# krullgit/3D-Object-Detection-for-autonomous-navigation

Measured on AMD Instinct MI355X. Metric: frames/sec (whole node) + p50 per-frame ms, 16k-pt pillars, higher is better.
Workload: dtype f32 (GEMMs on the 16-bit matrix pipe as split operands -- two float16 pieces per value, 3 products, fp32 accumulate: fp32-equivalent results, measured 1.5e-6 max from the fp32 oracle at this shape)

## Files before the change

### 3d-object-detection-for-autonomous-navigation_amd/csrc/backbone.hip

```cpp
#include <stdio.h>
#include <stdlib.h>
#include <string.h>

#include "pp_common.h"
#include "pp_plan.h"

typedef float f32x16 __attribute__((ext_vector_type(16)));
typedef _Float16 f16x8 __attribute__((ext_vector_type(8)));
#define PC_MFMA(A, B, C) __builtin_amdgcn_mfma_f32_32x32x16_f16(A, B, C, 0, 0, 0)
#define PC_PRODUCTS(ACC, XH, XM, YH, YM) \
    ACC = PC_MFMA(XM, YH, ACC); ACC = PC_MFMA(XH, YM, ACC); ACC = PC_MFMA(XH, YH, ACC);
typedef unsigned u32x4 __attribute__((ext_vector_type(4)));

__device__ __forceinline__ float4 buf_load16(__amdgpu_buffer_rsrc_t r, unsigned voff, unsigned soff) {
    const u32x4 v = __builtin_amdgcn_raw_buffer_load_b128(r, voff, soff, 0);
    return make_float4(__uint_as_float(v.x), __uint_as_float(v.y), __uint_as_float(v.z), __uint_as_float(v.w));
}
__device__ __forceinline__ void buf_store16(float4 v, __amdgpu_buffer_rsrc_t r, unsigned voff, unsigned soff) {
    const u32x4 u = {__float_as_uint(v.x), __float_as_uint(v.y), __float_as_uint(v.z), __float_as_uint(v.w)};
    __builtin_amdgcn_raw_buffer_store_b128(u, r, voff, soff, 0);
}
__device__ __forceinline__ __amdgpu_buffer_rsrc_t make_rsrc(const void* base) {
    return __builtin_amdgcn_make_buffer_rsrc(const_cast<void*>(base), 0, 0x7ffffffe, 0x00020000);
}

#define PX_TILE 128

#define KC 32
#define LDS_STRIDE 36

struct GemmArgs {
    const float* in;
    const float* dw;
    const float* wt;
    const unsigned short* wt16;
    int n_total;
    const float* bias;
    float* out;
    float* head;
    const float* head_wt;
    const float* head_wt16;
    const float* head_bias;
    int head_mode;
    int M;
    int tile_lo;
    int in_h, in_w, cin;
    int px_h, px_w;
    int stride;
    int ld_out, co_off;
    int epi;
    int k, cout;
    const int* occ;
    int occ_nz;
    const unsigned long long* occbits;
    int occ_w64;
    float* cls_plane;
    int cls_col0, cls_ncol;
    const float4* tr_coef;
    float* tr_D;
    float* tr_stat;
};

template <int NTILES>
__device__ __forceinline__ void gemm_epilogue(const GemmArgs& a, f32x16 (&acc)[NTILES], int p0, int n0, int wave,
                                              int lane, const int* s_opix) {
    const int h = lane >> 5, col_l = lane & 31;
    if (a.epi == 0) {
#pragma unroll
        for (int n = 0; n < NTILES; ++n) {
            const int col = n0 + n * 32 + col_l;
            const float bv = a.bias[col];
            float* dst = a.out + a.co_off + col;
#pragma unroll
            for (int r = 0; r < 16; ++r) {
                const int pix = p0 + wave * 32 + (r & 3) + 8 * (r >> 2) + 4 * h;
                if (pix < a.M) dst[(size_t)pix * a.ld_out] = relu_keep_nan(acc[n][r] + bv);
            }
        }
    } else if (a.epi == 1) {
        const int k = a.k, OW = a.px_w * k;
#pragma unroll
        for (int n = 0; n < NTILES; ++n) {
            const int col0 = __builtin_amdgcn_readfirstlane(n0 + n * 32);
            const int tap = col0 / a.cout, co = col0 - tap * a.cout + col_l;
            const int i = tap / k, j = tap - i * k;
            const int delta = i * OW + j;
            const float bv = a.bias[co];
            float* dst = a.out + a.co_off + co;
#pragma unroll
            for (int r = 0; r < 16; ++r) {
                const int row = wave * 32 + (r & 3) + 8 * (r >> 2) + 4 * h;
                if (p0 + row < a.M) dst[(size_t)(s_opix[row] + delta) * a.ld_out] = relu_keep_nan(acc[n][r] + bv);
            }
        }
    } else {
        const int col = n0 + col_l;
        const float bv = a.bias[col];
#pragma unroll
        for (int r = 0; r < 16; ++r) {
            const int pix = p0 + wave * 32 + (r & 3) + 8 * (r >> 2) + 4 * h;
            if (pix < a.M) a.head[(size_t)pix * PP_HEAD_COLS + col] = acc[0][r] + bv;
        }
    }
}

template <int NT, int MODE>
__global__ __launch_bounds__(256) void k_gemm_layer(GemmArgs a) {
    __shared__ __attribute__((aligned(16))) float sA[PX_TILE * LDS_STRIDE];
    __shared__ __attribute__((aligned(16))) float sB[NT * LDS_STRIDE];
    __shared__ int s_opix[PX_TILE];
    constexpr int NTILES = NT / 32;

    const int tid = threadIdx.x, lane = tid & 63, wave = tid >> 6;
    int mt;
    {
        const int nwg = gridDim.x, orig = blockIdx.x;
        const int q = nwg >> 3, r = nwg & 7, xcd = orig & 7;
        mt = ((xcd < r) ? xcd * (q + 1) : r * (q + 1) + (xcd - r) * q) + (orig >> 3);
    }
    const int p0 = mt * PX_TILE;
    const int n0 = blockIdx.y * NT;
    const int cin = a.cin;
    if (a.epi == 1 && tid < PX_TILE) {
        const int pix = min(p0 + tid, a.M - 1);
        const int hw = a.px_h * a.px_w;
        const int b = pix / hw, rem = pix - b * hw;
        const int y = rem / a.px_w, x = rem - y * a.px_w;
        s_opix[tid] = (b * a.px_h * a.k + y * a.k) * (a.px_w * a.k) + x * a.k;
    }

    const int c4 = tid & 7;
    const float* ibase[4];
    int yi0[4], xi0[4];
    bool pvalid[4];
    {
        const int hw = a.px_h * a.px_w;
#pragma unroll
        for (int it = 0; it < 4; ++it) {
            const int pix = p0 + (tid >> 3) + 32 * it;
            pvalid[it] = pix < a.M;
            const int pc = pvalid[it] ? pix : 0;
            const int b = pc / hw;
            const int rem = pc - b * hw;
            const int yo = rem / a.px_w, xo = rem - yo * a.px_w;
            if (MODE == 0) {
                yi0[it] = yo * a.stride - 1;
                xi0[it] = xo * a.stride - 1;
                ibase[it] = a.in + (size_t)b * a.in_h * a.in_w * cin;
            } else {
                yi0[it] = 0; xi0[it] = 0;
                ibase[it] = a.in + (size_t)pc * cin;
            }
        }
    }

    f32x16 acc[NTILES];
#pragma unroll
    for (int n = 0; n < NTILES; ++n)
#pragma unroll
        for (int r = 0; r < 16; ++r) acc[n][r] = 0.f;
// ... 1315 lines not shown
}

template <int NT, int WPS>
__global__ __launch_bounds__(256, WPS) void k_deconv_u(GemmArgs a, int ntiles) {
    constexpr int KCH = 16;
    constexpr int NTILES = NT / 32;
    constexpr int SB = PP_NPIECE * NT * 8;
    constexpr int NBI = NT * 2 * PP_NPIECE;
    constexpr int NB4 = (NBI + 255) / 256;
    constexpr int SHW = (NT / 16) * PP_NPIECE * 32 * 8;
    __shared__ __attribute__((aligned(16))) float sB[2 * SB];
    __shared__ __attribute__((aligned(16))) float sHW[SHW];
    __shared__ float s_bias[NT];
    __shared__ float s_hbias[PP_HEAD_COLS];
    __shared__ int s_opix[2][128];
    const int tid = threadIdx.x, lane = tid & 63, wave = tid >> 6;
    const int h = lane >> 5, r32 = lane & 31;

    const int xcd = blockIdx.x & 7, gl = blockIdx.x >> 3, GL = gridDim.x >> 3;
    const int tbase = (int)(((long long)xcd * ntiles) >> 3), tend = (int)(((long long)(xcd + 1) * ntiles) >> 3);
    const int first = tbase + gl;
    if (first >= tend) return;
    const int ntl = (tend - first + GL - 1) / GL;
    const int n0 = blockIdx.y * NT;
    const int cin = a.cin;
    const int nchunks = cin / KCH;
    const int total = ntl * nchunks;
    const int tap = n0 / a.cout, cbase = n0 - tap * a.cout;
    const int ti = tap / a.k;
    const int delta = ti * (a.px_w * a.k) + (tap - ti * a.k);
    const bool heads = a.head_mode != 0;

    const int hwpx = a.px_h * a.px_w;
#define D_FILL_OPIX(TILE, SLOT)                                                         \
    if (tid < 128) {                                                                    \
        const int pix_ = min((TILE) * 128 + tid, a.M - 1);                              \
        const int b_ = pix_ / hwpx, rem_ = pix_ - b_ * hwpx;                            \
        const int y_ = rem_ / a.px_w, x_ = rem_ - y_ * a.px_w;                          \
        s_opix[SLOT][tid] = (b_ * a.px_h * a.k + y_ * a.k) * (a.px_w * a.k) + x_ * a.k; \
    }
    D_FILL_OPIX(first, 0)

    const __amdgpu_buffer_rsrc_t rs_in = make_rsrc(reinterpret_cast<const char*>(a.in) - PP_ZPAD_FLOATS * 4);
    const __amdgpu_buffer_rsrc_t rs_wt = make_rsrc(a.wt16);
    unsigned boff[NB4];
    int bdst[NB4];
#pragma unroll
    for (int r = 0; r < NB4; ++r) {
        const int e_ = (tid + 256 * r) % NBI;
        const int piece = e_ / (NT * 2), rem = e_ % (NT * 2), row = rem >> 1, half = rem & 1;
        boff[r] = (unsigned)(((piece * a.n_total + n0 + row) * 16 + half * 8) * 2);
        bdst[r] = piece * (NT * 8) + row * 8 + ((half ^ ((row >> 3) & 1)) * 4);
    }
    const unsigned bstep = (unsigned)(PP_NPIECE * a.n_total * 32);
    float4 rb0, rb1, rb2;
    rb0 = rb1 = rb2 = make_float4(0.f, 0.f, 0.f, 0.f);
    static_assert(NB4 <= 3, "weight prefetch registers");
#define D_LOAD_B(KCIDX)                                                                                  \
    {                                                                                                    \
        const unsigned sb_ = (unsigned)(KCIDX) * bstep;                                                  \
        if (NBI % 256 == 0 || NB4 > 1 || tid < NBI) rb0 = buf_load16(rs_wt, boff[0], sb_);               \
        if (NB4 > 1 && (NBI >= 512 || tid + 256 < NBI)) rb1 = buf_load16(rs_wt, boff[NB4 > 1 ? 1 : 0], sb_);  \
        if (NB4 > 2 && (NBI >= 768 || tid + 512 < NBI)) rb2 = buf_load16(rs_wt, boff[NB4 > 2 ? 2 : 0], sb_);  \
    }
#define D_STORE_B(BUF)                                                                                   \
    {                                                                                                    \
        if (NBI % 256 == 0 || NB4 > 1 || tid < NBI) *reinterpret_cast<float4*>(sB + (BUF) * SB + bdst[0]) = rb0;  \
        if (NB4 > 1 && (NBI >= 512 || tid + 256 < NBI)) *reinterpret_cast<float4*>(sB + (BUF) * SB + bdst[NB4 > 1 ? 1 : 0]) = rb1;  \
        if (NB4 > 2 && (NBI >= 768 || tid + 512 < NBI)) *reinterpret_cast<float4*>(sB + (BUF) * SB + bdst[NB4 > 2 ? 2 : 0]) = rb2;  \
    }
    int ld_tile = first, ld_kc = 0;
    unsigned avo = 0;
#define D_TILE_AOFF(TILE)                                                                                \
    {                                                                                                    \
        const int pix_ = (TILE) * 128 + wave * 32 + r32;                                                 \
        avo = (pix_ < a.M) ? (unsigned)(pix_ * cin + h * 8) * 4u + PP_ZPAD_FLOATS * 4u : (unsigned)(h * 32);  \
    }
#define D_LOAD_A(R0, R1)                                                                                 \
    {                                                                                                    \
        if (ld_kc == 0) D_TILE_AOFF(ld_tile)                                                             \
        const unsigned so_ = (unsigned)ld_kc * (KCH * 4);                                                \
        R0 = buf_load16(rs_in, avo, so_);                                                                \
        R1 = buf_load16(rs_in, avo + 16u, so_);                                                          \
        if (++ld_kc == nchunks) { ld_kc = 0; ld_tile += GL; }                                            \
    }
    float4 ra0, ra1, rc0, rc1;
    D_LOAD_A(ra0, ra1)
    D_LOAD_A(rc0, rc1)
    D_LOAD_B(0)
    int lb_kc = 1;
    if (tid < NT) s_bias[tid] = a.bias[cbase + tid];
    if (heads) {
        for (int e = tid; e < SHW / 4; e += 256)
            reinterpret_cast<float4*>(sHW)[e ^ ((e >> 4) & 1)] = reinterpret_cast<const float4*>(a.head_wt16)[e];
        if (tid < PP_HEAD_COLS) s_hbias[tid] = a.head_bias[tid];
    }

    int mm_tile = first, mm_kc = 0, mm_slot = 0;
    __syncthreads();
    f32x16 acc[NTILES];
#define D_INIT_ACC()                                                                                     \
    _Pragma("unroll") for (int n = 0; n < NTILES; ++n)                                                   \
        _Pragma("unroll") for (int r = 0; r < 16; ++r) acc[n][r] = s_bias[n * 32 + DCH(r, h)];
    D_INIT_ACC()
    D_STORE_B(0)
    D_LOAD_B(lb_kc)
    if (++lb_kc == nchunks) lb_kc = 0;
    __syncthreads();

#define D_STEP(I, RA0, RA1)                                                                              \
    {                                                                                                    \
        const int i_ = (I);                                                                              \
        const float av_[8] = {RA0.x, RA0.y, RA0.z, RA0.w, RA1.x, RA1.y, RA1.z, RA1.w};                   \
        f16x8 ah_, am_;                                                                                  \
        split_f16x2(av_, ah_, am_);                                                                      \
        if (i_ + 2 < total) D_LOAD_A(RA0, RA1)                                                           \
        {                                                                                                \
            const float* cB_ = sB + (i_ & 1) * SB + r32 * 8 + ((h ^ ((r32 >> 3) & 1)) * 4);              \
            _Pragma("unroll") for (int n = 0; n < NTILES; ++n) {                                         \
                const f16x8 bh_ = *reinterpret_cast<const f16x8*>(cB_ + n * 32 * 8);                     \
                const f16x8 bm_ = *reinterpret_cast<const f16x8*>(cB_ + NT * 8 + n * 32 * 8);            \
                PC_PRODUCTS(acc[n], bh_, bm_, ah_, am_)                                                  \
            }                                                                                            \
        }                                                                                                \
        if (i_ + 1 < total) D_STORE_B((i_ + 1) & 1)              \
        if (++mm_kc == nchunks) {                                                                        \
            deconv_tile_epilogue<NT>(a, acc, mm_tile, wave, lane, cbase, delta, s_opix[mm_slot], sHW, s_hbias);  \
            D_INIT_ACC()                                                                                 \
            mm_kc = 0;                                                                                   \
            mm_tile += GL;                                                                               \
            mm_slot ^= 1;                                                                                \
        } else if (mm_kc == 1 && mm_tile + GL < tend) {                                                  \
            D_FILL_OPIX(mm_tile + GL, mm_slot ^ 1)           \
        }                                                                                                \
        if (i_ + 1 < total) {    \
            if (i_ + 2 < total) D_LOAD_B(lb_kc)                                                          \
            if (++lb_kc == nchunks) lb_kc = 0;                                                           \
        }                                                                                                \
        __syncthreads();                                                                                 \
    }
    for (int i = 0; i < total; i += 2) {
        D_STEP(i, ra0, ra1)
        D_STEP(i + 1, rc0, rc1)
    }
#undef D_STEP
#undef D_INIT_ACC
#undef D_LOAD_A
#undef D_TILE_AOFF
#undef D_STORE_B
#undef D_LOAD_B
#undef D_FILL_OPIX
}

template <int CIN>
__global__ __launch_bounds__(256, 2) void k_deconv_r(GemmArgs a, int nunits, int upw) {
    constexpr int NCH = CIN / 16;
    constexpr int STEPS = 4 * NCH;
    constexpr int NPU = STEPS / 8;
    constexpr int PANEL = 8 * 2 * 256;
    constexpr int NB = 3;
    constexpr int PD = 2;
    constexpr int SHW = (128 / 16) * 2 * 32 * 8;
    static_assert(STEPS % 4 == 0 && PD < 4, "fragment ring of four");
    __shared__ __attribute__((aligned(16))) float sW[NB * PANEL];
    __shared__ __attribute__((aligned(16))) float sHW[SHW];
    __shared__ __attribute__((aligned(16))) float s_bias[128];
    __shared__ float s_hbias[PP_HEAD_COLS];
    const int tid = threadIdx.x, lane = tid & 63, wave = __builtin_amdgcn_readfirstlane(tid >> 6);
    const int h = lane >> 5, r32 = lane & 31;

    int wg;
    {
        const int G = gridDim.x, q = G >> 3, r = G & 7, xcd = blockIdx.x & 7;
        wg = (xcd < r ? xcd * (q + 1) : r * (q + 1) + (xcd - r) * q) + (blockIdx.x >> 3);
    }
    const int u0 = wg * upw, u1 = min(u0 + upw, nunits);
    if (u0 >= u1) return;
    const int ntaps = a.k * a.k;
    const bool heads = a.head_mode != 0;
    const int hwpx = a.px_h * a.px_w, OW = a.px_w * a.k;

    const __amdgpu_buffer_rsrc_t rs_in = make_rsrc(reinterpret_cast<const char*>(a.in) - PP_ZPAD_FLOATS * 4);
    const __amdgpu_buffer_rsrc_t rs_wt = make_rsrc(a.wt16);
    const int srow = lane >> 1, shalf = lane & 1;
    const unsigned wvoff = (unsigned)((((wave & 1) * a.n_total + srow) * 16 + shalf * 8) * 2);
    const int wdst = wave * 256 + srow * 8 + ((shalf ^ ((srow >> 3) & 1)) * 4);
    const unsigned cstep = (unsigned)(2 * a.n_total * 32);
    float4 rw[4];
    rw[0] = rw[1] = rw[2] = rw[3] = make_float4(0.f, 0.f, 0.f, 0.f);
    int tile = u0 / ntaps, tap = u0 - tile * ntaps;
    int ld_left = (u1 - u0) * NPU, ld_tap = tap, ld_p = 0;
#define R_LOAD_NEXT()                                                                                    \
    {                                                                                                    \
        if (ld_left > 0) {                                                                               \
            _Pragma("unroll") for (int j_ = 0; j_ < 4; ++j_) {                                           \
                const int fs_ = ld_p * 8 + (wave >> 1) + 2 * j_;                                         \
                const int nt_ = fs_ / NCH, c_ = fs_ % NCH;                                               \
                rw[j_] = buf_load16(rs_wt, wvoff, (unsigned)c_ * cstep + (unsigned)((ld_tap * 128 + nt_ * 32) * 32)); \
            }                                                                                            \
        }                                                                                                \
        --ld_left;                                                                                       \
        if (++ld_p == NPU) { ld_p = 0; if (++ld_tap == ntaps) ld_tap = 0; }                              \
    }
#define R_STORE_W(SLOT)                                                                                  \
    _Pragma("unroll") for (int j_ = 0; j_ < 4; ++j_)                                                     \
        *reinterpret_cast<float4*>(sW + (SLOT) * PANEL + wdst + j_ * 1024) = rw[j_];

    float4 ra0[NCH][2];
    const int pix0_ = tile * 128 + wave * 32 + r32;
    const bool ok0_ = pix0_ < a.M;
    {
        const unsigned avo = ok0_ ? (unsigned)(pix0_ * CIN + h * 8) * 4u + PP_ZPAD_FLOATS * 4u : (unsigned)(h * 32);
#pragma unroll
        for (int c = 0; c < NCH; ++c) {
            ra0[c][0] = buf_load16(rs_in, avo, (unsigned)c * 64u);
            ra0[c][1] = buf_load16(rs_in, avo + 16u, (unsigned)c * 64u);
        }
    }
    R_LOAD_NEXT()
    for (int e = tid; e < 128; e += 256) s_bias[e] = a.bias[e];
    if (heads) {
        for (int e = tid; e < SHW / 4; e += 256)
            reinterpret_cast<float4*>(sHW)[e ^ ((e >> 4) & 1)] = reinterpret_cast<const float4*>(a.head_wt16)[e];
        if (tid < PP_HEAD_COLS) s_hbias[tid] = a.head_bias[tid];
    }
    R_STORE_W(0)
    R_LOAD_NEXT()
    __syncthreads();

    f16x8 xh[NCH], xm[NCH];
    int tile_cur = tile, opix0;
    bool ok = ok0_;
    {
        const int pc = ok ? pix0_ : 0;
        const int pb = pc / hwpx, prem = pc - pb * hwpx;
        const int py = prem / a.px_w, pxx = prem - py * a.px_w;
        opix0 = (pb * a.px_h * a.k + py * a.k) * OW + pxx * a.k;
#pragma unroll
        for (int c = 0; c < NCH; ++c) {
            const float av[8] = {ra0[c][0].x, ra0[c][0].y, ra0[c][0].z, ra0[c][0].w, ra0[c][1].x, ra0[c][1].y, ra0[c][1].z, ra0[c][1].w};
            split_f16x2(av, xh[c], xm[c]);
        }
    }
    const float* const cW = sW + r32 * 8 + ((h ^ ((r32 >> 3) & 1)) * 4);
    const float* const cHW = sHW + r32 * 8 + ((h ^ ((r32 >> 3) & 1)) * 4);
    int slot = 0;
    const float* pcur = cW;
    const float* pnxt = cW + PANEL;
    f16x8 fh[4], fm[4];
#pragma unroll
    for (int i = 0; i < PD; ++i) {
        fh[i] = *reinterpret_cast<const f16x8*>(pcur + i * 512);
        fm[i] = *reinterpret_cast<const f16x8*>(pcur + i * 512 + 256);
    }

    constexpr bool PREF = CIN <= 128;
    float4 rn[PREF ? NCH : 1][2];
    int pre_tile = -1;
    for (int u = u0; u < u1; ++u) {
        if (tile != tile_cur) {
            tile_cur = tile;
            const int pix = tile * 128 + wave * 32 + r32;
            ok = pix < a.M;
            const unsigned avo = ok ? (unsigned)(pix * CIN + h * 8) * 4u + PP_ZPAD_FLOATS * 4u : (unsigned)(h * 32);
            float4 ra[NCH][2];
            if (PREF && pre_tile == tile) {
#pragma unroll
                for (int c = 0; c < NCH; ++c) { ra[c][0] = rn[PREF ? c : 0][0]; ra[c][1] = rn[PREF ? c : 0][1]; }
            } else {
#pragma unroll
                for (int c = 0; c < NCH; ++c) {
                    ra[c][0] = buf_load16(rs_in, avo, (unsigned)c * 64u);
                    ra[c][1] = buf_load16(rs_in, avo + 16u, (unsigned)c * 64u);
                }
            }
            const int pc = ok ? pix : 0;
            const int pb = pc / hwpx, prem = pc - pb * hwpx;
            const int py = prem / a.px_w, pxx = prem - py * a.px_w;
            opix0 = (pb * a.px_h * a.k + py * a.k) * OW + pxx * a.k;
#pragma unroll
            for (int c = 0; c < NCH; ++c) {
                const float av[8] = {ra[c][0].x, ra[c][0].y, ra[c][0].z, ra[c][0].w, ra[c][1].x, ra[c][1].y, ra[c][1].z, ra[c][1].w};
                split_f16x2(av, xh[c], xm[c]);
            }
        }
        const int ti = tap / a.k;
        const size_t orow = (size_t)(opix0 + ti * OW + (tap - ti * a.k));
        float* const hrow = a.head + orow * PP_HEAD_COLS + 4 * h;
        f32x16 hacc;
        if (a.head_mode == 2 && ok) {
#pragma unroll
            for (int g = 0; g < 4; ++g) {
                const float4 t = *reinterpret_cast<const float4*>(hrow + 8 * g);
                hacc[4 * g] = t.x; hacc[4 * g + 1] = t.y; hacc[4 * g + 2] = t.z; hacc[4 * g + 3] = t.w;
            }
        } else {
#pragma unroll
            for (int r = 0; r < 16; ++r) hacc[r] = (a.head_mode == 1) ? s_hbias[DCH(r, h)] : 0.f;
        }
        float* const dst = (a.out != nullptr) ? a.out + orow * a.ld_out + a.co_off + 4 * h : nullptr;
        f32x16 acc;
        __builtin_amdgcn_sched_barrier(0);
#pragma unroll
        for (int fs = 0; fs < STEPS; ++fs) {
            const int s = fs & 7, nt = fs / NCH, c = fs % NCH;
            if (c == 0) {
#pragma unroll
                for (int g = 0; g < 4; ++g) {
                    const float4 t = *reinterpret_cast<const float4*>(s_bias + nt * 32 + 8 * g + 4 * h);
                    acc[4 * g] = t.x; acc[4 * g + 1] = t.y; acc[4 * g + 2] = t.z; acc[4 * g + 3] = t.w;
                }
            }
            if (s == 4) __syncthreads();
            {
                const float* w_ = (s + PD < 8) ? pcur + (s + PD) * 512 : pnxt + (s + PD - 8) * 512;
                fh[(fs + PD) & 3] = *reinterpret_cast<const f16x8*>(w_);
                fm[(fs + PD) & 3] = *reinterpret_cast<const f16x8*>(w_ + 256);
            }
            PC_PRODUCTS(acc, fh[fs & 3], fm[fs & 3], xh[c], xm[c])
            if (s == 0) {
                const int ws = (slot + 1 == NB) ? 0 : slot + 1;
                R_STORE_W(ws)
            }
            if (s == 1) { R_LOAD_NEXT() }
            if (PREF && fs == 1 && tap + 1 == ntaps && u + 1 < u1) {
                pre_tile = tile + 1;
                const int pixn = pre_tile * 128 + wave * 32 + r32;
                const unsigned avn = (pixn < a.M) ? (unsigned)(pixn * CIN + h * 8) * 4u + PP_ZPAD_FLOATS * 4u : (unsigned)(h * 32);
#pragma unroll
                for (int c = 0; c < (PREF ? NCH : 0); ++c) {
                    rn[c][0] = buf_load16(rs_in, avn, (unsigned)c * 64u);
                    rn[c][1] = buf_load16(rs_in, avn + 16u, (unsigned)c * 64u);
                }
            }
            if (s == 7) {
                slot = (slot + 1 == NB) ? 0 : slot + 1;
                pcur = pnxt;
                pnxt = cW + ((slot + 1 == NB) ? 0 : slot + 1) * PANEL;
            }
            __builtin_amdgcn_sched_barrier(0);
            if (c == NCH - 1) {
                float v[16];
#pragma unroll
                for (int r = 0; r < 16; ++r) v[r] = relu_keep_nan(acc[r]);
                if (heads) {
#pragma unroll
                    for (int g = 0; g < 2; ++g) {
                        const float av[8] = {v[8 * g], v[8 * g + 1], v[8 * g + 2], v[8 * g + 3],
                                             v[8 * g + 4], v[8 * g + 5], v[8 * g + 6], v[8 * g + 7]};
                        f16x8 yh, ym;
                        split_f16x2(av, yh, ym);
                        const float* hW = cHW + (nt * 2 + g) * 2 * 32 * 8;
                        const f16x8 gh = *reinterpret_cast<const f16x8*>(hW);
                        const f16x8 gm = *reinterpret_cast<const f16x8*>(hW + 32 * 8);
                        PC_PRODUCTS(hacc, gh, gm, yh, ym)
                    }
                }
                if (dst != nullptr && ok) {
#pragma unroll
                    for (int g = 0; g < 4; ++g)
                        *reinterpret_cast<float4*>(dst + nt * 32 + 8 * g) = make_float4(v[4 * g], v[4 * g + 1], v[4 * g + 2], v[4 * g + 3]);
                }
                __builtin_amdgcn_sched_barrier(0);
            }
        }
        if (heads && ok) {
#pragma unroll
            for (int g = 0; g < 4; ++g)
                *reinterpret_cast<float4*>(hrow + 8 * g) = make_float4(hacc[4 * g], hacc[4 * g + 1], hacc[4 * g + 2], hacc[4 * g + 3]);
            if (a.cls_plane != nullptr) {
                float* cp = a.cls_plane + orow * a.cls_ncol;
#pragma unroll
                for (int r = 0; r < 16; ++r) {
                    const int col = 8 * (r >> 2) + 4 * h + (r & 3) - a.cls_col0;
                    if ((unsigned)col < (unsigned)a.cls_ncol) cp[col] = hacc[r];
                }
            }
        }
        if (++tap == ntaps) { tap = 0; ++tile; }
    }
#undef R_STORE_W
#undef R_LOAD_NEXT
}

template <int CIN>
static void launch_deconv_r(const GemmArgs& a, int cus, hipStream_t s) {
    const int ntiles = (a.M + 127) / 128;
    const long long U = (long long)ntiles * a.k * a.k;
    const int slots = 2 * cus;
    const int upw = (int)((U + slots - 1) / slots);
    const int G = (int)((U + upw - 1) / upw);
    PP_LAUNCH("k_deconv_r", (k_deconv_r<CIN>), dim3((unsigned)G), dim3(256), 0, s, a, (int)U, upw);
}

template <int NT>
__global__ __launch_bounds__(256, 2) void k_deconv_k4(GemmArgs a) {
    constexpr int KCH = 16;
    constexpr int NTILES = NT / 32;
    constexpr int SB = PP_NPIECE * NT * 8;
    constexpr int NBL = NT * 2 * PP_NPIECE / 64;
    constexpr int SHW = (NT / 16) * PP_NPIECE * 32 * 8;
    constexpr int SLOT = 16 * 64;
    constexpr int OWNERS = NTILES < 4 ? NTILES : 4;
    constexpr int SR = (4 * SB > (4 * NTILES - OWNERS) * SLOT) ? 4 * SB : (4 * NTILES - OWNERS) * SLOT;
    __shared__ __attribute__((aligned(16))) float sR[SR];
    __shared__ __attribute__((aligned(16))) float sHW[SHW];
    __shared__ float s_bias[NT];
    __shared__ float s_hbias[PP_HEAD_COLS];
    const int tid = threadIdx.x, lane = tid & 63, wave = tid >> 6;
    const int h = lane >> 5, r32 = lane & 31;
    const int n0 = blockIdx.y * NT;
    const int cin = a.cin;
    const int niter = cin / (KCH * 4);
    const int tap = n0 / a.cout, cbase = n0 - tap * a.cout;
    const int ti = tap / a.k;
    const int delta = ti * (a.px_w * a.k) + (tap - ti * a.k);
    const bool heads = a.head_mode != 0;
    float* const sBw = sR + wave * SB;

    const __amdgpu_buffer_rsrc_t rs_in = make_rsrc(reinterpret_cast<const char*>(a.in) - PP_ZPAD_FLOATS * 4);
    const __amdgpu_buffer_rsrc_t rs_wt = make_rsrc(a.wt16);
    const int pix = blockIdx.x * 32 + r32;
    const bool ok = pix < a.M;
    const unsigned avo = ok ? (unsigned)(pix * cin + h * 8) * 4u + PP_ZPAD_FLOATS * 4u : (unsigned)(h * 32);
    float4 ra[4][2];
#pragma unroll
    for (int j = 0; j < 4; ++j) {
        ra[j][0] = ra[j][1] = make_float4(0.f, 0.f, 0.f, 0.f);
        if (j < niter) {
            const unsigned so = (unsigned)(wave + 4 * j) * (KCH * 4);
            ra[j][0] = buf_load16(rs_in, avo, so);
            ra[j][1] = buf_load16(rs_in, avo + 16u, so);
        }
    }
    unsigned boff[NBL];
    int bdst[NBL];
#pragma unroll
    for (int r = 0; r < NBL; ++r) {
        const int e = lane + 64 * r;
        const int piece = e / (NT * 2), rem = e % (NT * 2), row = rem >> 1, half = rem & 1;
        boff[r] = (unsigned)(((piece * a.n_total + n0 + row) * 16 + half * 8) * 2);
        bdst[r] = piece * (NT * 8) + row * 8 + ((half ^ ((row >> 3) & 1)) * 4);
    }
    const unsigned bstep = (unsigned)(PP_NPIECE * a.n_total * 32);
    float4 rb[NBL];
#pragma unroll
    for (int r = 0; r < NBL; ++r) rb[r] = buf_load16(rs_wt, boff[r], (unsigned)wave * bstep);
    if (tid < NT) s_bias[tid] = a.bias[cbase + tid];
    if (heads) {
        for (int e = tid; e < SHW / 4; e += 256)
            reinterpret_cast<float4*>(sHW)[e ^ ((e >> 4) & 1)] = reinterpret_cast<const float4*>(a.head_wt16)[e];
        if (tid < PP_HEAD_COLS) s_hbias[tid] = a.head_bias[tid];
    }
    f32x16 acc[NTILES];
#pragma unroll
    for (int n = 0; n < NTILES; ++n)
#pragma unroll
        for (int r = 0; r < 16; ++r) acc[n][r] = 0.f;
    const float* const cB = sBw + r32 * 8 + ((h ^ ((r32 >> 3) & 1)) * 4);
#pragma unroll
    for (int j = 0; j < 4; ++j) {
        if (j < niter) {
#pragma unroll
            for (int r = 0; r < NBL; ++r) *reinterpret_cast<float4*>(sBw + bdst[r]) = rb[r];
            if (j + 1 < niter) {
#pragma unroll
                for (int r = 0; r < NBL; ++r) rb[r] = buf_load16(rs_wt, boff[r], (unsigned)(wave + 4 * (j + 1)) * bstep);
            }
            const float av[8] = {ra[j][0].x, ra[j][0].y, ra[j][0].z, ra[j][0].w, ra[j][1].x, ra[j][1].y, ra[j][1].z, ra[j][1].w};
            f16x8 ah, am;
            split_f16x2(av, ah, am);
#pragma unroll
            for (int n = 0; n < NTILES; ++n) {
                const f16x8 bh = *reinterpret_cast<const f16x8*>(cB + n * 32 * 8);
                const f16x8 bm = *reinterpret_cast<const f16x8*>(cB + NT * 8 + n * 32 * 8);
                PC_PRODUCTS(acc[n], bh, bm, ah, am)
            }
        }
    }
    auto slot = [](int w, int n) -> int {
        return w * NTILES + n - (w < OWNERS ? w : OWNERS) - ((w < OWNERS && n > w) ? 1 : 0);
    };
    __syncthreads();
#pragma unroll
    for (int n = 0; n < NTILES; ++n)
        if (n != wave) {
            float* d = sR + slot(wave, n) * SLOT + lane * 4;
#pragma unroll
            for (int g = 0; g < 4; ++g)
                *reinterpret_cast<float4*>(d + g * 256) = make_float4(acc[n][4 * g], acc[n][4 * g + 1], acc[n][4 * g + 2], acc[n][4 * g + 3]);
        }
    __syncthreads();
    const int pc = ok ? pix : 0;
    const int hwpx = a.px_h * a.px_w;
    const int pb = pc / hwpx, prem = pc - pb * hwpx;
    const int py = prem / a.px_w, pxx = prem - py * a.px_w;
    const size_t orow = (size_t)((pb * a.px_h * a.k + py * a.k) * (a.px_w * a.k) + pxx * a.k + delta);
    f32x16 hpart;
#pragma unroll
    for (int r = 0; r < 16; ++r) hpart[r] = 0.f;
    if (wave < NTILES) {
        float v[16];
#pragma unroll
        for (int n = 0; n < NTILES; ++n)
            if (n == wave) {
#pragma unroll
                for (int r = 0; r < 16; ++r) v[r] = acc[n][r];
            }
#pragma unroll
        for (int w = 0; w < 4; ++w)
            if (w != wave) {
                const float* sp = sR + slot(w, wave) * SLOT + lane * 4;
#pragma unroll
                for (int g = 0; g < 4; ++g) {
                    const float4 t = *reinterpret_cast<const float4*>(sp + g * 256);
                    v[4 * g] += t.x; v[4 * g + 1] += t.y; v[4 * g + 2] += t.z; v[4 * g + 3] += t.w;
                }
            }
#pragma unroll
        for (int r = 0; r < 16; ++r) v[r] = relu_keep_nan(v[r] + s_bias[wave * 32 + DCH(r, h)]);
        if (a.out != nullptr && ok) {
            float* dst = a.out + orow * a.ld_out + a.co_off + cbase + 4 * h + wave * 32;
#pragma unroll
            for (int g = 0; g < 4; ++g)
                *reinterpret_cast<float4*>(dst + 8 * g) = make_float4(v[4 * g], v[4 * g + 1], v[4 * g + 2], v[4 * g + 3]);
        }
        if (heads) {
#pragma unroll
            for (int g = 0; g < 2; ++g) {
                const float av[8] = {v[8 * g], v[8 * g + 1], v[8 * g + 2], v[8 * g + 3],
                                     v[8 * g + 4], v[8 * g + 5], v[8 * g + 6], v[8 * g + 7]};
                f16x8 xh, xm;
                split_f16x2(av, xh, xm);
// ... 189 lines not shown
```

Before: 92320.

## Switch deconv kernel from 32x32x16 to 16x16x32 MFMA fragments

Rewrites k_deconv_r's inner GEMM and head GEMM to use 16x16x32 f16 MFMAs instead of 32x32x16. Each wave now processes two 16-pixel halves, and the weight staging, LDS layout, input loads, head-weight shuffle and output/head/cls stores are remapped to the new fragment layout. The aim is a cheaper or better-scheduled MFMA shape with smaller accumulators, which may also relieve register pressure. The cost is more complex index math and twice as many MFMA issues, and every store path is remapped, so a layout error would be easy to make.

```diff
diff --git a/3d-object-detection-for-autonomous-navigation_amd/csrc/backbone.hip b/3d-object-detection-for-autonomous-navigation_amd/csrc/backbone.hip
--- a/3d-object-detection-for-autonomous-navigation_amd/csrc/backbone.hip
+++ b/3d-object-detection-for-autonomous-navigation_amd/csrc/backbone.hip
@@ -6,6 +6,7 @@
 #include "pp_plan.h"
 
 typedef float f32x16 __attribute__((ext_vector_type(16)));
+typedef float f32x4 __attribute__((ext_vector_type(4)));
 typedef _Float16 f16x8 __attribute__((ext_vector_type(8)));
 #define PC_MFMA(A, B, C) __builtin_amdgcn_mfma_f32_32x32x16_f16(A, B, C, 0, 0, 0)
 #define PC_PRODUCTS(ACC, XH, XM, YH, YM) \
@@ -1627,6 +1628,11 @@
 #undef D_FILL_OPIX
 }
 
+#define PC_MFMA16(A, B, C) __builtin_amdgcn_mfma_f32_16x16x32_f16(A, B, C, 0, 0, 0)
+#define PC_PRODUCTS16(P0, P1, WH, WM, X0H, X0M, X1H, X1M)                      \
+    P0 = PC_MFMA16(WM, X0H, P0); P1 = PC_MFMA16(WM, X1H, P1);                  \
+    P0 = PC_MFMA16(WH, X0M, P0); P1 = PC_MFMA16(WH, X1M, P1);                  \
+    P0 = PC_MFMA16(WH, X0H, P0); P1 = PC_MFMA16(WH, X1H, P1);
 template <int CIN>
 __global__ __launch_bounds__(256, 2) void k_deconv_r(GemmArgs a, int nunits, int upw) {
     constexpr int NCH = CIN / 16;
@@ -1635,14 +1641,15 @@
     constexpr int PANEL = 8 * 2 * 256;
     constexpr int NB = 3;
     constexpr int PD = 2;
-    constexpr int SHW = (128 / 16) * 2 * 32 * 8;
+    constexpr int SHW = 4 * 2 * 2 * 256;
     static_assert(STEPS % 4 == 0 && PD < 4, "fragment ring of four");
     __shared__ __attribute__((aligned(16))) float sW[NB * PANEL];
     __shared__ __attribute__((aligned(16))) float sHW[SHW];
     __shared__ __attribute__((aligned(16))) float s_bias[128];
-    __shared__ float s_hbias[PP_HEAD_COLS];
+    __shared__ __attribute__((aligned(16))) float s_hbias[PP_HEAD_COLS];
     const int tid = threadIdx.x, lane = tid & 63, wave = __builtin_amdgcn_readfirstlane(tid >> 6);
-    const int h = lane >> 5, r32 = lane & 31;
+    const int p16 = lane & 15, q = lane >> 4;
+    const int crow = 16 * (q >> 1) + 4 * (q & 1);
 
     int wg;
     {
@@ -1657,10 +1664,10 @@
 
     const __amdgpu_buffer_rsrc_t rs_in = make_rsrc(reinterpret_cast<const char*>(a.in) - PP_ZPAD_FLOATS * 4);
     const __amdgpu_buffer_rsrc_t rs_wt = make_rsrc(a.wt16);
-    const int srow = lane >> 1, shalf = lane & 1;
-    const unsigned wvoff = (unsigned)((((wave & 1) * a.n_total + srow) * 16 + shalf * 8) * 2);
-    const int wdst = wave * 256 + srow * 8 + ((shalf ^ ((srow >> 3) & 1)) * 4);
     const unsigned cstep = (unsigned)(2 * a.n_total * 32);
+    const int srow = 16 * (p16 >> 3) + 8 * ((wave >> 1) & 1) + (p16 & 7);
+    const unsigned wvoff = (unsigned)((((wave & 1) * a.n_total + srow) * 16 + (q & 1) * 8) * 2) + (unsigned)(q >> 1) * cstep;
+    const int wdst = wave * 256 + lane * 4;
     float4 rw[4];
     rw[0] = rw[1] = rw[2] = rw[3] = make_float4(0.f, 0.f, 0.f, 0.f);
     int tile = u0 / ntaps, tap = u0 - tile * ntaps;
@@ -1671,7 +1678,7 @@
             _Pragma("unroll") for (int j_ = 0; j_ < 4; ++j_) {                                           \
                 const int fs_ = ld_p * 8 + (wave >> 1) + 2 * j_;                                         \
                 const int nt_ = fs_ / NCH, c_ = fs_ % NCH;                                               \
-                rw[j_] = buf_load16(rs_wt, wvoff, (unsigned)c_ * cstep + (unsigned)((ld_tap * 128 + nt_ * 32) * 32)); \
+                rw[j_] = buf_load16(rs_wt, wvoff, (unsigned)(c_ & ~1) * cstep + (unsigned)((ld_tap * 128 + nt_ * 32) * 32)); \
             }                                                                                            \
         }                                                                                                \
         --ld_left;                                                                                       \
@@ -1681,22 +1688,41 @@
     _Pragma("unroll") for (int j_ = 0; j_ < 4; ++j_)                                                     \
         *reinterpret_cast<float4*>(sW + (SLOT) * PANEL + wdst + j_ * 1024) = rw[j_];
 
+#define R_TILE_PIXELS(TILE, OKV, AVO, OPIX)                                                              \
+    _Pragma("unroll") for (int ph_ = 0; ph_ < 2; ++ph_) {                                                \
+        const int pix_ = (TILE) * 128 + wave * 32 + ph_ * 16 + p16;                                      \
+        OKV[ph_] = pix_ < a.M;                                                                           \
+        AVO[ph_] = OKV[ph_] ? (unsigned)(pix_ * CIN + q * 8) * 4u + PP_ZPAD_FLOATS * 4u : (unsigned)(q * 32); \
+        const int pc_ = OKV[ph_] ? pix_ : 0;                                                             \
+        const int pb_ = pc_ / hwpx, prem_ = pc_ - pb_ * hwpx;                                            \
+        const int py_ = prem_ / a.px_w, pxx_ = prem_ - py_ * a.px_w;                                     \
+        OPIX[ph_] = (pb_ * a.px_h * a.k + py_ * a.k) * OW + pxx_ * a.k;                                  \
+    }
+#define R_LOAD_INPUT(RA, AVO)                                                                            \
+    _Pragma("unroll") for (int c_ = 0; c_ < NCH; ++c_) {                                                 \
+        RA[c_][0] = buf_load16(rs_in, AVO[c_ & 1], (unsigned)(c_ >> 1) * 128u);                          \
+        RA[c_][1] = buf_load16(rs_in, AVO[c_ & 1] + 16u, (unsigned)(c_ >> 1) * 128u);                    \
+    }
+#define R_SPLIT_INPUT(RA)                                                                                \
+    _Pragma("unroll") for (int c_ = 0; c_ < NCH; ++c_) {                                                 \
+        const float av_[8] = {RA[c_][0].x, RA[c_][0].y, RA[c_][0].z, RA[c_][0].w,                        \
+                              RA[c_][1].x, RA[c_][1].y, RA[c_][1].z, RA[c_][1].w};                       \
+        split_f16x2(av_, xh[c_], xm[c_]);                                                                \
+    }
     float4 ra0[NCH][2];
-    const int pix0_ = tile * 128 + wave * 32 + r32;
-    const bool ok0_ = pix0_ < a.M;
-    {
-        const unsigned avo = ok0_ ? (unsigned)(pix0_ * CIN + h * 8) * 4u + PP_ZPAD_FLOATS * 4u : (unsigned)(h * 32);
-#pragma unroll
-        for (int c = 0; c < NCH; ++c) {
-            ra0[c][0] = buf_load16(rs_in, avo, (unsigned)c * 64u);
-            ra0[c][1] = buf_load16(rs_in, avo + 16u, (unsigned)c * 64u);
-        }
-    }
+    bool ok[2];
+    unsigned avo0[2];
+    int opix0[2];
+    R_TILE_PIXELS(tile, ok, avo0, opix0)
+    R_LOAD_INPUT(ra0, avo0)
     R_LOAD_NEXT()
     for (int e = tid; e < 128; e += 256) s_bias[e] = a.bias[e];
     if (heads) {
-        for (int e = tid; e < SHW / 4; e += 256)
-            reinterpret_cast<float4*>(sHW)[e ^ ((e >> 4) & 1)] = reinterpret_cast<const float4*>(a.head_wt16)[e];
+        for (int e = tid; e < SHW / 4; e += 256) {
+            const int l = e & 63, piece = (e >> 6) & 1, ch = (e >> 7) & 1, nt = e >> 8, lq = l >> 4;
+            const int src = (((2 * nt + (lq >> 1)) * 2 + piece) * PP_HEAD_COLS + 16 * ch + (l & 15)) * 2 + (lq & 1);
+            reinterpret_cast<float4*>(sHW)[e] = reinterpret_cast<const float4*>(a.head_wt16)[src];
+        }
         if (tid < PP_HEAD_COLS) s_hbias[tid] = a.head_bias[tid];
     }
     R_STORE_W(0)
@@ -1704,21 +1730,10 @@
     __syncthreads();
 
     f16x8 xh[NCH], xm[NCH];
-    int tile_cur = tile, opix0;
-    bool ok = ok0_;
-    {
-        const int pc = ok ? pix0_ : 0;
-        const int pb = pc / hwpx, prem = pc - pb * hwpx;
-        const int py = prem / a.px_w, pxx = prem - py * a.px_w;
-        opix0 = (pb * a.px_h * a.k + py * a.k) * OW + pxx * a.k;
-#pragma unroll
-        for (int c = 0; c < NCH; ++c) {
-            const float av[8] = {ra0[c][0].x, ra0[c][0].y, ra0[c][0].z, ra0[c][0].w, ra0[c][1].x, ra0[c][1].y, ra0[c][1].z, ra0[c][1].w};
-            split_f16x2(av, xh[c], xm[c]);
-        }
-    }
-    const float* const cW = sW + r32 * 8 + ((h ^ ((r32 >> 3) & 1)) * 4);
-    const float* const cHW = sHW + r32 * 8 + ((h ^ ((r32 >> 3) & 1)) * 4);
+    int tile_cur = tile;
+    R_SPLIT_INPUT(ra0)
+    const float* const cW = sW + lane * 4;
+    const float* const cHW = sHW + lane * 4;
     int slot = 0;
     const float* pcur = cW;
     const float* pnxt = cW + PANEL;
@@ -1735,55 +1750,47 @@
     for (int u = u0; u < u1; ++u) {
         if (tile != tile_cur) {
             tile_cur = tile;
-            const int pix = tile * 128 + wave * 32 + r32;
-            ok = pix < a.M;
-            const unsigned avo = ok ? (unsigned)(pix * CIN + h * 8) * 4u + PP_ZPAD_FLOATS * 4u : (unsigned)(h * 32);
+            unsigned avo[2];
+            R_TILE_PIXELS(tile, ok, avo, opix0)
             float4 ra[NCH][2];
             if (PREF && pre_tile == tile) {
 #pragma unroll
                 for (int c = 0; c < NCH; ++c) { ra[c][0] = rn[PREF ? c : 0][0]; ra[c][1] = rn[PREF ? c : 0][1]; }
             } else {
-#pragma unroll
-                for (int c = 0; c < NCH; ++c) {
-                    ra[c][0] = buf_load16(rs_in, avo, (unsigned)c * 64u);
-                    ra[c][1] = buf_load16(rs_in, avo + 16u, (unsigned)c * 64u);
+                R_LOAD_INPUT(ra, avo)
+            }
+            R_SPLIT_INPUT(ra)
+        }
+        const int ti = tap / a.k;
+        const int toff = ti * OW + (tap - ti * a.k);
+#define R_OROW(PH) ((size_t)(opix0[PH] + toff))
+#define R_HROW(PH) (a.head + R_OROW(PH) * PP_HEAD_COLS + 4 * q)
+        f32x4 hacc[2][2];
+#pragma unroll
+        for (int ph = 0; ph < 2; ++ph) {
+#pragma unroll
+            for (int ch = 0; ch < 2; ++ch) {
+                if (a.head_mode == 2 && ok[ph]) {
+                    const float4 t = *reinterpret_cast<const float4*>(R_HROW(ph) + 16 * ch);
+                    hacc[ch][ph] = f32x4{t.x, t.y, t.z, t.w};
+                } else if (a.head_mode == 1) {
+                    const float4 t = *reinterpret_cast<const float4*>(s_hbias + 16 * ch + 4 * q);
+                    hacc[ch][ph] = f32x4{t.x, t.y, t.z, t.w};
+                } else {
+                    hacc[ch][ph] = f32x4{0.f, 0.f, 0.f, 0.f};
                 }
             }
-            const int pc = ok ? pix : 0;
-            const int pb = pc / hwpx, prem = pc - pb * hwpx;
-            const int py = prem / a.px_w, pxx = prem - py * a.px_w;
-            opix0 = (pb * a.px_h * a.k + py * a.k) * OW + pxx * a.k;
-#pragma unroll
-            for (int c = 0; c < NCH; ++c) {
-                const float av[8] = {ra[c][0].x, ra[c][0].y, ra[c][0].z, ra[c][0].w, ra[c][1].x, ra[c][1].y, ra[c][1].z, ra[c][1].w};
-                split_f16x2(av, xh[c], xm[c]);
-            }
-        }
-        const int ti = tap / a.k;
-        const size_t orow = (size_t)(opix0 + ti * OW + (tap - ti * a.k));
-        float* const hrow = a.head + orow * PP_HEAD_COLS + 4 * h;
-        f32x16 hacc;
-        if (a.head_mode == 2 && ok) {
-#pragma unroll
-            for (int g = 0; g < 4; ++g) {
-                const float4 t = *reinterpret_cast<const float4*>(hrow + 8 * g);
-                hacc[4 * g] = t.x; hacc[4 * g + 1] = t.y; hacc[4 * g + 2] = t.z; hacc[4 * g + 3] = t.w;
-            }
-        } else {
-#pragma unroll
-            for (int r = 0; r < 16; ++r) hacc[r] = (a.head_mode == 1) ? s_hbias[DCH(r, h)] : 0.f;
-        }
-        float* const dst = (a.out != nullptr) ? a.out + orow * a.ld_out + a.co_off + 4 * h : nullptr;
-        f32x16 acc;
+        }
+        f32x4 acc[2][2];
         __builtin_amdgcn_sched_barrier(0);
 #pragma unroll
         for (int fs = 0; fs < STEPS; ++fs) {
-            const int s = fs & 7, nt = fs / NCH, c = fs % NCH;
+            const int s = fs & 7, nt = fs / NCH, c = fs % NCH, x0 = c & ~1, rh = c & 1;
             if (c == 0) {
 #pragma unroll
-                for (int g = 0; g < 4; ++g) {
-                    const float4 t = *reinterpret_cast<const float4*>(s_bias + nt * 32 + 8 * g + 4 * h);
-                    acc[4 * g] = t.x; acc[4 * g + 1] = t.y; acc[4 * g + 2] = t.z; acc[4 * g + 3] = t.w;
+                for (int r = 0; r < 2; ++r) {
+                    const float4 t = *reinterpret_cast<const float4*>(s_bias + nt * 32 + 8 * r + crow);
+                    acc[r][0] = acc[r][1] = f32x4{t.x, t.y, t.z, t.w};
                 }
             }
             if (s == 4) __syncthreads();
@@ -1792,7 +1799,7 @@
                 fh[(fs + PD) & 3] = *reinterpret_cast<const f16x8*>(w_);
                 fm[(fs + PD) & 3] = *reinterpret_cast<const f16x8*>(w_ + 256);
             }
-            PC_PRODUCTS(acc, fh[fs & 3], fm[fs & 3], xh[c], xm[c])
+            PC_PRODUCTS16(acc[rh][0], acc[rh][1], fh[fs & 3], fm[fs & 3], xh[x0], xm[x0], xh[x0 + 1], xm[x0 + 1])
             if (s == 0) {
                 const int ws = (slot + 1 == NB) ? 0 : slot + 1;
                 R_STORE_W(ws)
@@ -1800,12 +1807,12 @@
             if (s == 1) { R_LOAD_NEXT() }
             if (PREF && fs == 1 && tap + 1 == ntaps && u + 1 < u1) {
                 pre_tile = tile + 1;
-                const int pixn = pre_tile * 128 + wave * 32 + r32;
-                const unsigned avn = (pixn < a.M) ? (unsigned)(pixn * CIN + h * 8) * 4u + PP_ZPAD_FLOATS * 4u : (unsigned)(h * 32);
 #pragma unroll
                 for (int c = 0; c < (PREF ? NCH : 0); ++c) {
-                    rn[c][0] = buf_load16(rs_in, avn, (unsigned)c * 64u);
-                    rn[c][1] = buf_load16(rs_in, avn + 16u, (unsigned)c * 64u);
+                    const int pixn = pre_tile * 128 + wave * 32 + (c & 1) * 16 + p16;
+                    const unsigned avn = (pixn < a.M) ? (unsigned)(pixn * CIN + q * 8) * 4u + PP_ZPAD_FLOATS * 4u : (unsigned)(q * 32);
+                    rn[c][0] = buf_load16(rs_in, avn, (unsigned)(c >> 1) * 128u);
+                    rn[c][1] = buf_load16(rs_in, avn + 16u, (unsigned)(c >> 1) * 128u);
                 }
             }
             if (s == 7) {
@@ -1815,45 +1822,61 @@
             }
             __builtin_amdgcn_sched_barrier(0);
             if (c == NCH - 1) {
-                float v[16];
-#pragma unroll
-                for (int r = 0; r < 16; ++r) v[r] = relu_keep_nan(acc[r]);
+                float v[2][8];
+#pragma unroll
+                for (int ph = 0; ph < 2; ++ph)
+#pragma unroll
+                    for (int r = 0; r < 8; ++r) v[ph][r] = relu_keep_nan(acc[r >> 2][ph][r & 3]);
                 if (heads) {
-#pragma unroll
-                    for (int g = 0; g < 2; ++g) {
-                        const float av[8] = {v[8 * g], v[8 * g + 1], v[8 * g + 2], v[8 * g + 3],
-                                             v[8 * g + 4], v[8 * g + 5], v[8 * g + 6], v[8 * g + 7]};
-                        f16x8 yh, ym;
-                        split_f16x2(av, yh, ym);
-                        const float* hW = cHW + (nt * 2 + g) * 2 * 32 * 8;
+                    f16x8 yh[2], ym[2];
+                    split_f16x2(v[0], yh[0], ym[0]);
+                    split_f16x2(v[1], yh[1], ym[1]);
+#pragma unroll
+                    for (int ch = 0; ch < 2; ++ch) {
+                        const float* hW = cHW + (nt * 2 + ch) * 512;
                         const f16x8 gh = *reinterpret_cast<const f16x8*>(hW);
-                        const f16x8 gm = *reinterpret_cast<const f16x8*>(hW + 32 * 8);
-                        PC_PRODUCTS(hacc, gh, gm, yh, ym)
+                        const f16x8 gm = *reinterpret_cast<const f16x8*>(hW + 256);
+                        PC_PRODUCTS16(hacc[ch][0], hacc[ch][1], gh, gm, yh[0], ym[0], yh[1], ym[1])
                     }
                 }
-                if (dst != nullptr && ok) {
-#pragma unroll
-                    for (int g = 0; g < 4; ++g)
-                        *reinterpret_cast<float4*>(dst + nt * 32 + 8 * g) = make_float4(v[4 * g], v[4 * g + 1], v[4 * g + 2], v[4 * g + 3]);
+                if (a.out != nullptr) {
+#pragma unroll
+                    for (int ph = 0; ph < 2; ++ph)
+                        if (ok[ph]) {
+                            float* const dst = a.out + R_OROW(ph) * a.ld_out + a.co_off + crow + nt * 32;
+#pragma unroll
+                            for (int r = 0; r < 2; ++r)
+                                *reinterpret_cast<float4*>(dst + 8 * r) =
+                                    make_float4(v[ph][4 * r], v[ph][4 * r + 1], v[ph][4 * r + 2], v[ph][4 * r + 3]);
+                        }
                 }
                 __builtin_amdgcn_sched_barrier(0);
             }
         }
-        if (heads && ok) {
-#pragma unroll
-            for (int g = 0; g < 4; ++g)
-                *reinterpret_cast<float4*>(hrow + 8 * g) = make_float4(hacc[4 * g], hacc[4 * g + 1], hacc[4 * g + 2], hacc[4 * g + 3]);
-            if (a.cls_plane != nullptr) {
-                float* cp = a.cls_plane + orow * a.cls_ncol;
-#pragma unroll
-                for (int r = 0; r < 16; ++r) {
-                    const int col = 8 * (r >> 2) + 4 * h + (r & 3) - a.cls_col0;
-                    if ((unsigned)col < (unsigned)a.cls_ncol) cp[col] = hacc[r];
+#pragma unroll
+        for (int ph = 0; ph < 2; ++ph)
+            if (heads && ok[ph]) {
+#pragma unroll
+                for (int ch = 0; ch < 2; ++ch)
+                    *reinterpret_cast<float4*>(R_HROW(ph) + 16 * ch) =
+                        make_float4(hacc[ch][ph][0], hacc[ch][ph][1], hacc[ch][ph][2], hacc[ch][ph][3]);
+                if (a.cls_plane != nullptr) {
+                    const int col0 = 4 * q - a.cls_col0;
+                    const long long cp0 = (long long)R_OROW(ph) * a.cls_ncol + col0;
+#pragma unroll
+                    for (int r = 0; r < 8; ++r) {
+                        const int dc = 16 * (r >> 2) + (r & 3);
+                        if ((unsigned)(col0 + dc) < (unsigned)a.cls_ncol) a.cls_plane[cp0 + dc] = hacc[r >> 2][ph][r & 3];
+                    }
                 }
             }
-        }
         if (++tap == ntaps) { tap = 0; ++tile; }
-    }
+#undef R_HROW
+#undef R_OROW
+    }
+#undef R_SPLIT_INPUT
+#undef R_LOAD_INPUT
+#undef R_TILE_PIXELS
 #undef R_STORE_W
 #undef R_LOAD_NEXT
 }
```

Result: no change. 91650, median of 2 (-0.7%).
